# indrajeetadityaroy9/vit-inductive-bias-distillation

Hardware: AMD Instinct MI355X
Metric: distillation images/sec (BASD loss fwd+bwd+grad all-reduce), DeiT-S<-ResNet-50 @ bs256/GPU (higher is better)
Workload: dtype f32; 1 GPU; cfg2 DeiT-S<-ResNet-50 224x224; per_gpu_batch=256, global_batch=256, input_dtype=float32, layout=strided (CLS-sliced / channel-major views), backward=True, grad_allreduce_bytes=88202672, grad_allreduce=none at world size 1 (bucket packed, nothing to exchange), rank_readback=auto, readback_deferred_steps=1756, selector=basd_selector_chain mode 0, parallelism=dp1

## Files before the change

### include/basd_hip.h

```cpp
#ifndef BASD_HIP_H
#define BASD_HIP_H

#include <stdint.h>

#ifdef __cplusplus
extern "C" {
#endif

#ifndef __HIP_PLATFORM_AMD__
typedef struct ihipStream_t* hipStream_t;
#endif

#define BASD_OK 0
#define BASD_EINVAL (-1)
#define BASD_EUNSUPPORTED (-2)
#define BASD_DTYPE_F32 0
#define BASD_DTYPE_BF16 1


int basd_gemm_nt(const void* a, int a_dtype, long a_sb, long a_sn, long a_sd, int a_rows_per_batch,
                 long a_batch_stride, const float* b, long ldb, long b_batch_stride, int M, int N, int K, int batch,
                 float* c, long ldc, long c_batch_stride, float scale, const float* bias, float beta,
                 float* colsum_part, float* col_mean, hipStream_t stream);

// ... 10 lines not shown
                 int rows, int cols, int batch, int parts, float* partial, float* mean, hipStream_t stream);

int basd_gemm_tuning(int split_bf16);
int basd_gemm_tuning_get(void);

int basd_colmean_multi(const void* const* x_ptrs, int dtype, long sb, long sn, long sd, int rows_per_batch, int rows,
                       int cols, int n_mats, int parts, float* partial, float* means, int vec_ok,
                       hipStream_t stream);

int basd_syrk_splits(int krows, int cols, int n_mats);

int basd_syrk_multi(const void* const* x_ptrs, int dtype, long sb, long sn, long sd, int rows_per_batch, int krows,
                    int cols, int n_mats, const float* means, const float* scales, int splits, float* slabs,
                    float* out, long out_stride, int vec_ok, const float* fold, int fold_parts, int fold_from,
                    hipStream_t stream);


int basd_jacobi_workspace_ints(int batch, int max_sweeps);
int basd_jacobi_plain4_fits(int n);

int basd_jacobi_tuning(int lanes_per_pair);
int basd_jacobi_ordering(int odd_even);

int basd_jacobi_onesided(float* W, long batch_stride, int rows_dot, int rows_tot, int n, int batch,
                         const int* n_arr, float* colnorm, int colnorm_stride, int max_sweeps, float tol_cos,
                         int* flags, int* sweeps_out, hipStream_t stream);

long basd_jacobi_twopass_workspace_bytes(int n, int batch, int max_sweeps);
int basd_jacobi_stacked_twopass(float* W, long batch_stride, int n, int batch, float* colnorm, int colnorm_stride,
                                int max_sweeps, float tol_cos, void* workspace, int* sweeps_out, hipStream_t stream);
// ... 60 lines not shown
                              const unsigned* go_flag, unsigned go_value, int go_budget, hipStream_t stream);
int basd_flag_set(unsigned* flag, unsigned value, hipStream_t stream);

typedef struct BasdSelectorChain {
    const void* const* teacher_host_ptrs;
    long t_dtype, t_sb, t_sn, t_sd;
    const void* const* student_ptrs;
    long s_dtype, s_sb, s_sn, s_sd, s_vec_ok;
    const float* proj_t;
    const float* proj_s_t;
    long E, L, B, n_s, n_t, d_s, d_t;
    double mp_factor;
    long rank_cap;
    long kmax, kmax_cap, mode;
    float* z; float* z_sums; const void* const* z_ptrs; float* z_means; float* t_slabs; long t_splits;
    float* s_partial; float* s_means; float* s_slabs; long s_splits, s_parts;
    float* grams; float* d; float* e; float* tau; float* vh; float* vals; void* tri_work; void* tri_work_s;
    int* ranks; int* host_mirror;
    int* student_status_mirror;
    float* zv; float* vecs; float* u_rot; float* sw; float* cos; float* sigma; float* d_out;
    int* k_arr; const int* sw_index; int* jflags;
    hipStream_t main_stream, chain_stream, student_stream, tail_stream;
    void* ev_fork; void* ev_student; void* ev_ranks; void* ev_tail; void* ev_slot_free; void* ev_tgram; void* ev_tg0;
    long release_delay;
    hipStream_t fact_stream; unsigned* go_flag; long go_value; long go_budget;
    void* tm_proj; void* tm_tgram; void* tm_scol0; void* tm_scol1; void* tm_sgram; void* tm_tri0; void* tm_mid; void* tm_spec;
    hipStream_t cert_stream; int* cert_mirror; void* ev_cert;
    double* cert_scratch;
} BasdSelectorChain;
int basd_selector_chain(const BasdSelectorChain* args);
int basd_rank_certificate(const float* grams, const float* zbar, int n, int batch, double factor, double* scratch,
// ... 164 lines not shown
```

### vit-inductive-bias-distillation_amd/basd_amd/_lib.py

```python
from __future__ import annotations

import ctypes as C
import os
import threading

_HERE = os.path.dirname(os.path.abspath(__file__))
LIB_PATH = os.path.join(_HERE, "libbasd_hip.so")

vp, i32, i64, f32, f64 = C.c_void_p, C.c_int, C.c_long, C.c_float, C.c_double

SIGNATURES = {
    "basd_gemm_nt": [vp, i32, i64, i64, i64, i32, i64, vp, i64, i64, i32, i32, i32, i32, vp, i64, i64, f32, vp, f32,
                     vp, vp, vp],
    "basd_gemm_tn_splits": [i32],
    "basd_gemm_tn": [vp, vp, i32, i64, i64, i64, i64, i64, i64, i64, i64, i32, i32, i32, i32, i32, vp, vp, i32, vp,
                     vp, i64, i64, f32, vp],
    "basd_colmean_parts": [i32],
    "basd_colmean": [vp, i32, i64, i64, i64, i32, i64, i32, i32, i32, i32, vp, vp, vp],
    "basd_colmean_multi": [vp, i32, i64, i64, i64, i32, i32, i32, i32, i32, vp, vp, i32, vp],
    "basd_syrk_splits": [i32, i32, i32],
    "basd_syrk_multi": [vp, i32, i64, i64, i64, i32, i32, i32, i32, vp, vp, i32, vp, vp, i64, i32, vp, i32, i32, vp],
    "basd_jacobi_workspace_ints": [i32, i32],
    "basd_jacobi_twopass_workspace_bytes": [i32, i32, i32],
    "basd_jacobi_stacked_twopass": [vp, i64, i32, i32, vp, i32, i32, f32, vp, vp, vp],
    "basd_jacobi_tuning": [i32],
    "basd_jacobi_ordering": [i32],
    "basd_gemm_tuning": [i32],
    "basd_gemm_tuning_get": [],
    "basd_jacobi_onesided": [vp, i64, i32, i32, i32, i32, vp, vp, i32, i32, f32, vp, vp, vp],
    "basd_sort_extract": [vp, i64, i32, i32, i32, i32, vp, i32, vp, vp, i32, vp],
    "basd_tridiag_workspace_bytes": [i32, i32],
    "basd_tridiag_tuning": [i32, i32, i32, i32, i32, i32],
    "basd_tridiag": [vp, i64, i32, i32, vp, vp, vp, vp, vp, vp],
    "basd_tridiag_ranked": [vp, i64, i32, i32, vp, vp, vp, vp, vp, i32, f64, i32, vp, vp, vp, vp],
    "basd_tridiag_ranked_gated": [vp, i64, i32, i32, vp, vp, vp, vp, vp, i32, f64, i32, vp, vp, vp, C.c_uint, i32, vp],
    "basd_flag_set": [vp, C.c_uint, vp],
# ... 83 lines not shown
                             "grad_layers", "g_slabs")]
        + [("g_splits", i64)]
        + [("uw_ce", vp), ("uw_out", vp), ("jac_ws", vp), ("w_stack", vp), ("sigma_u", vp)]
    )


class SelectorChainArgs(C.Structure):
    _fields_ = (
        [("teacher_host_ptrs", vp)] + [(n, i64) for n in ("t_dtype", "t_sb", "t_sn", "t_sd")]
        + [("student_ptrs", vp)] + [(n, i64) for n in ("s_dtype", "s_sb", "s_sn", "s_sd", "s_vec_ok")]
        + [("proj_t", vp), ("proj_s_t", vp)]
        + [(n, i64) for n in ("E", "L", "B", "n_s", "n_t", "d_s", "d_t")]
        + [("mp_factor", f64)]
        + [(n, i64) for n in ("rank_cap", "kmax", "kmax_cap", "mode")]
        + [(n, vp) for n in ("z", "z_sums", "z_ptrs", "z_means", "t_slabs")] + [("t_splits", i64)]
        + [(n, vp) for n in ("s_partial", "s_means", "s_slabs")] + [("s_splits", i64), ("s_parts", i64)]
        + [(n, vp) for n in ("grams", "d", "e", "tau", "vh", "vals", "tri_work", "tri_work_s", "ranks", "host_mirror",
                             "student_status_mirror", "zv", "vecs", "u_rot", "sw", "cos", "sigma", "d_out", "k_arr",
                             "sw_index", "jflags", "main_stream", "chain_stream", "student_stream", "tail_stream",
                             "ev_fork", "ev_student", "ev_ranks", "ev_tail", "ev_slot_free", "ev_tgram", "ev_tg0",
                             "release_delay", "fact_stream", "go_flag", "go_value", "go_budget",
                             "tm_proj", "tm_tgram", "tm_scol0", "tm_scol1", "tm_sgram", "tm_tri0", "tm_mid", "tm_spec",
                             "cert_stream", "cert_mirror", "ev_cert", "cert_scratch")]
    )


EINVAL, EUNSUPPORTED = -1, -2

LONG_RESULTS = {"basd_tridiag_workspace_bytes", "basd_jacobi_twopass_workspace_bytes",
                "basd_mix_grad_tokens_scratch_floats", "basd_teacher_center_stream_scratch_floats",
                "basd_rank_certificate_scratch_bytes"}
# ... 47 lines not shown
```

### vit-inductive-bias-distillation_amd/basd_amd/chain.py

```python
from __future__ import annotations

import ctypes as C

import torch

from . import _lib, ops

import os

RELEASE_DELAY = int(os.environ.get("BASD_CHAIN_RELEASE_DELAY", "0"))
EARLY_LAUNCH = os.environ.get("BASD_CHAIN_EARLY", "0") == "1"
EARLY_BUDGET = 1500
CERTIFICATE = os.environ.get("BASD_RANK_CERT", "1") != "0"
SLOTS = max(2, int(os.environ.get("BASD_CHAIN_SLOTS", "3")))
TAIL_STREAMS = int(os.environ.get("BASD_TAIL_STREAMS", "0"))
TAIL_SPLIT_RANK = 96
SPEC_MARGIN = 8


TIMED_EVENTS = False
TM_NAMES = ("tm_proj", "tm_tgram", "tm_scol0", "tm_scol1", "tm_sgram", "tm_tri0", "tm_mid", "tm_spec")
TIMING: list | None = None


# ... 13 lines not shown
class _Slot:

    def __init__(self, plan: "SelectorChainPlan"):
        p = plan
        dev, f32, i32 = p.device, torch.float32, torch.int32
        E, L, n, K = p.E, p.L, p.d_s, p.kmax_cap
        M_t, M_s = p.B * p.n_t, p.B * p.n_s
        tiles = (M_t + 127) // 128
        nmat = 2 * L + E

        def buf(count, dtype=f32):
            return torch.empty((int(count),), device=dev, dtype=dtype)

        self.t_splits = _lib.query("basd_syrk_splits", M_t, n, L)
        self.s_splits = _lib.query("basd_syrk_splits", M_s, n, E)
        self.s_parts = _lib.query("basd_colmean_parts", M_s)
        b = self.bufs = dict(
            z=buf(L * M_t * n), z_sums=buf(L * tiles * n), z_means=buf(L * n), t_slabs=buf(L * self.t_splits * n * n),
            s_partial=buf(E * self.s_parts * n), s_means=buf(E * n), s_slabs=buf(E * self.s_splits * n * n),
            grams=buf(nmat * n * n), d=buf(nmat * n), e=buf(nmat * n), tau=buf(nmat * n), vh=buf(nmat * n * n),
            vals=buf(nmat * n), ranks=buf(L, i32),
            zv=buf((L + E) * K * n), vecs=buf((L + E) * K * n), u_rot=buf(L * K * n), sw=buf(L * K),
            cos=buf(E * L * K * K), sigma=buf(E * L * K), k_arr=buf(E * L, i32),
            jflags=buf(_lib.query("basd_jacobi_workspace_ints", E * L, ops.MAX_SWEEPS), i32),
        )
        split = p.mode not in (0, 4)
        b["tri_work"] = buf(_lib.query("basd_tridiag_workspace_bytes", n, 2 * L if split else nmat), torch.uint8)
        b["tri_work_s"] = buf(_lib.query("basd_tridiag_workspace_bytes", n, E), torch.uint8) if split else None
        b["z_ptrs"] = torch.tensor([b["z"].data_ptr() + 4 * l * M_t * n for l in range(L)], dtype=torch.int64).to(dev)
        b["sw_index"] = torch.tensor(list(range(L)) * E, dtype=i32).to(dev)
        b["go_flag"] = torch.zeros((1,), device=dev, dtype=i32)
        self.go_value = 0
        self.mirror = torch.zeros((L + 8,), dtype=i32).pin_memory()
        self.student_mirror = torch.zeros((8,), dtype=i32).pin_memory() if split else None
        self.ev_fork, self.ev_student, self.ev_ranks, self.ev_tail, self.ev_tgram, self.ev_tg0 = (_event() for _ in range(6))
        self.ev_cert = _event()
        self.cert_mirror = torch.zeros((8,), dtype=i32).pin_memory()
        self.used = False
        self.student_status_pending = False
        self.teacher_ptrs = (C.c_void_p * L)()
        self.d_out = None

        a = self.args = _lib.SelectorChainArgs()
        a.teacher_host_ptrs = C.cast(self.teacher_ptrs, C.c_void_p)
        a.E, a.L, a.B, a.n_s, a.n_t, a.d_s, a.d_t = E, L, p.B, p.n_s, p.n_t, n, p.d_t
        a.mp_factor = (1 + (n / M_t) ** 0.5) ** 2
        a.rank_cap, a.kmax_cap, a.mode = n - 1, K, p.mode
        a.t_splits, a.s_splits, a.s_parts = self.t_splits, self.s_splits, self.s_parts
        for name in ("z", "z_sums", "z_ptrs", "z_means", "t_slabs", "s_partial", "s_means", "s_slabs", "grams", "d", "e",
                     "tau", "vh", "vals", "tri_work", "tri_work_s", "ranks", "zv", "vecs", "u_rot", "sw", "cos", "sigma",
                     "k_arr", "sw_index", "jflags"):
            setattr(a, name, None if b[name] is None else b[name].data_ptr())
        a.host_mirror = self.mirror.data_ptr()
        a.student_status_mirror = None if self.student_mirror is None else self.student_mirror.data_ptr()
        a.ev_fork, a.ev_student, a.ev_ranks, a.ev_tail = self.ev_fork, self.ev_student, self.ev_ranks, self.ev_tail
        a.ev_tgram = self.ev_tgram
        a.ev_tg0 = self.ev_tg0
        a.release_delay = RELEASE_DELAY
        if p.cert_stream is not None:
            b["cert_scratch"] = torch.zeros((_lib.query("basd_rank_certificate_scratch_bytes", L),), device=dev,
                                            dtype=torch.uint8)
            a.cert_stream, a.cert_mirror, a.ev_cert = p.cert_stream.cuda_stream, self.cert_mirror.data_ptr(), self.ev_cert
            a.cert_scratch = b["cert_scratch"].data_ptr()
# ... 127 lines not shown
```

### vit-inductive-bias-distillation_amd/basd_amd/ops.py

```python
from __future__ import annotations

from dataclasses import dataclass
from functools import lru_cache

import torch

from . import _lib

import os

F32, BF16 = 0, 1
MAX_SWEEPS = 20
TWO_PASS_SVD = True
TRANSPOSED_MIX_GRAD = True
TWO_PASS_LOG_LIMIT = 16 << 30
EIG_SOLVER = os.environ.get("BASD_EIG_SOLVER", "tridiag")
if os.environ.get("BASD_GEMM_SPLIT") in ("0", "1"):
    _lib.call("basd_gemm_tuning", int(os.environ["BASD_GEMM_SPLIT"]))
if os.environ.get("BASD_JACOBI_ORDERING") in ("0", "1"):
    _lib.call("basd_jacobi_ordering", int(os.environ["BASD_JACOBI_ORDERING"]))


def _stream() -> int:
    return torch._C._cuda_getCurrentRawStream(torch._C._cuda_getDevice())
# ... 143 lines not shown
        if len(_COLMEAN_SCRATCH) >= 16:
            _COLMEAN_SCRATCH.clear()
        partial = _COLMEAN_SCRATCH[key] = torch.empty((n, parts, cols), device=dev, dtype=torch.float32)
    _lib.call("basd_colmean_multi", table.data_ptr(), dt, sb, sn, sd, rpb, rows, cols, n, parts, partial.data_ptr(),
              means.data_ptr(), vec_ok, _stream())
    return means.view(n, cols)


def centered_grams(xs: list[torch.Tensor], *, centered: list[bool] | None = None,
                   scales: list[float] | None = None, out: torch.Tensor | None = None,
                   splits: int | None = None, means: torch.Tensor | None = None,
                   fold: tuple[torch.Tensor, int] | None = None) -> tuple[torch.Tensor, torch.Tensor]:
    (dt, sb, sn, sd, rpb), rows, cols, vec_ok = _gram_layout(xs)
    n, dev = len(xs), xs[0].device
    table = _ptr_table(xs)
    if fold is not None:
        part, fold_from = fold
        assert part.is_contiguous() and part.dtype == torch.float32 and part.shape[0] == n - fold_from
        means_used = None
        centered = None
    elif means is None:
        means = column_means(xs)
    if fold is not None:
        pass
    elif centered is not None and not all(centered):
        keep = _device_consts(tuple(1.0 if c else 0.0 for c in centered), torch.float32, dev)
        means_used = means * keep.unsqueeze(1)
    else:
        means_used = means
    sc = None
# ... 594 lines not shown
```

### vit-inductive-bias-distillation_amd/csrc/chain.hip

```cpp
#include "basd_common.h"
#include "../../include/basd_hip.h"
#include <stdlib.h>

namespace basd {

__global__ void __launch_bounds__(256) chain_sw_kernel(const float* __restrict__ vals, int n, int kmax,
                                                       float* __restrict__ sw) {
    const int l = blockIdx.x;
    for (int i = threadIdx.x; i < kmax; i += 256) sw[(long)l * kmax + i] = sqrtf(fmaxf(vals[(long)l * n + i], 0.f));
}

__global__ void chain_k_arr_kernel(const int* __restrict__ ranks, int L, int items, int kmax, int* __restrict__ k_arr) {
    const int i = blockIdx.x * blockDim.x + threadIdx.x;
    if (i < items) {
        int k = ranks[i % L];
        k = k < 1 ? 1 : k;
        k_arr[i] = k > kmax ? kmax : k;
    }
}

constexpr int CERT_BLOCKS = 32;
__global__ void __launch_bounds__(256) rank_certificate_kernel(const float* __restrict__ grams, const float* __restrict__ zbar,
                                                               int n, int L, double factor, double* __restrict__ scratch,
                                                               int* __restrict__ host_flag) {
// ... 244 lines not shown
    }
    BASD_TRY(basd_syrk_multi(a->z_ptrs, BASD_DTYPE_F32, 0, n, 1, 1 << 30, (int)M_t, n, L, a->z_means, nullptr,
                             (int)a->t_splits, a->t_slabs, a->grams + (long)L * nn, nn, 1, nullptr, 0, 0, cs));
    BASD_TRY(basd_gram_finish(a->grams + (long)L * nn, a->z_means, n, L, M_t, a->grams, nullptr, cs));
    BASD_MARK(a->tm_tgram, cs);
    if (mode == 3) BASD_CHECK_ARG(a->ev_tg0 != nullptr);
    if (a->ev_tg0) BASD_HIP(hipEventRecord((hipEvent_t)a->ev_tg0, cs));
    if (a->cert_mirror) {
        BASD_CHECK_ARG(a->cert_stream && a->ev_cert && a->ev_tg0 && a->cert_scratch);
        if (a->cert_stream != cs) BASD_HIP(hipStreamWaitEvent(a->cert_stream, (hipEvent_t)a->ev_tg0, 0));
        BASD_TRY(basd_rank_certificate(a->grams, a->z_means, n, L, a->mp_factor, a->cert_scratch, a->cert_mirror, a->cert_stream));
        BASD_HIP(hipEventRecord((hipEvent_t)a->ev_cert, a->cert_stream));
    }

    auto student_grams = [&](hipStream_t st) -> int {
        BASD_MARK(a->tm_scol0, st);
        BASD_TRY(basd_colmean_multi(a->student_ptrs, (int)a->s_dtype, a->s_sb, a->s_sn, a->s_sd, n_s, (int)M_s, n, E,
                                    (int)a->s_parts, a->s_partial, a->s_means, (int)a->s_vec_ok, st));
        BASD_MARK(a->tm_scol1, st);
        BASD_TRY(basd_syrk_multi(a->student_ptrs, (int)a->s_dtype, a->s_sb, a->s_sn, a->s_sd, n_s, (int)M_s, n, E,
                                 a->s_means, nullptr, (int)a->s_splits, a->s_slabs, a->grams + 2L * L * nn, nn,
                                 (int)a->s_vec_ok, nullptr, 0, 0, st));
        BASD_MARK(a->tm_sgram, st);
        return BASD_OK;
    };

    if (mode == 0 || mode == 4) {
        BASD_TRY(student_grams(ss));
        if (ss != cs) {
            BASD_HIP(hipEventRecord((hipEvent_t)a->ev_student, ss));
            BASD_HIP(hipStreamWaitEvent(cs, (hipEvent_t)a->ev_student, 0));
        }
        BASD_MARK(a->tm_tri0, cs);
        BASD_TRY(basd_tridiag_ranked(a->grams, nn, n, 2 * L + E, a->d, a->e, a->tau, a->vh, a->tri_work, L, a->mp_factor,
                                     (int)a->rank_cap, a->ranks, a->host_mirror, a->tm_mid, cs));
        BASD_HIP(hipEventRecord((hipEvent_t)a->ev_ranks, cs));
    } else {
// ... 29 lines not shown
```

### vit-inductive-bias-distillation_amd/csrc/gemm.hip

```cpp
#include "basd_common.h"

namespace basd {

typedef float f32x16 __attribute__((ext_vector_type(16)));

constexpr int BM = 128, BN = 128;

typedef __bf16 bf16x8 __attribute__((ext_vector_type(8)));

__device__ __forceinline__ unsigned cvt_pk_bf16(float a, float b) {
    unsigned r;
    asm("v_cvt_pk_bf16_f32 %0, %1, %2" : "=v"(r) : "v"(a), "v"(b));
    return r;
}

__device__ __forceinline__ void split3(float a, float b, unsigned& hi, unsigned& mid, unsigned& lo) {
    hi = cvt_pk_bf16(a, b);
    const float ra = a - __uint_as_float(hi << 16), rb = b - __uint_as_float(hi & 0xffff0000u);
    mid = cvt_pk_bf16(ra, rb);
    const float sa = ra - __uint_as_float(mid << 16), sb = rb - __uint_as_float(mid & 0xffff0000u);
    lo = cvt_pk_bf16(sa, sb);
}


// ... 519 lines not shown
                    acc[mi][ni] = __builtin_amdgcn_mfma_f32_32x32x2f32(a[mi].w, b[ni].w, acc[mi][ni], 0, 0, 0);
                }
        }
    }
    store_tile(C, ldc, M, N, m0, n0, acc, wm, wn, lane, scale);
}


__device__ __forceinline__ void tri_tile(int p, int& mi, int& ni) {
    mi = 0;
    while ((mi + 1) * (mi + 2) / 2 <= p) ++mi;
    ni = p - mi * (mi + 1) / 2;
}

template <typename T, bool VEC>
__global__ void __launch_bounds__(256) syrk_tn_kernel(const void* const* __restrict__ ptrs, GemmOperand X, int cols,
                                                      int Krows, int splits, int n_mats, int pairs,
                                                      const float* __restrict__ means, float* __restrict__ slabs,
                                                      const float* __restrict__ fold, int fold_parts, int fold_from) {
    __shared__ __attribute__((aligned(16))) float lds[2 * TN_BK * 128];
    int pair, unit;
    {
        const int units = splits * n_mats, id = blockIdx.x;
        if ((units & 7) == 0) {
            const int xcd = id & 7, slot = id >> 3;
            pair = slot % pairs;
            unit = xcd + 8 * (slot / pairs);
        } else {
            pair = id % pairs;
            unit = id / pairs;
        }
    }
    int tmi, tni;
    tri_tile(pair, tmi, tni);
// ... 26 lines not shown
    const int col0 = is_b ? n0 : m0;
    float* tile = is_b ? tB : tA;
    float reg[2][4][4], m4[4];
    TnCursor cu;
    tn_cursor_init(cu, X, k_begin, t);
    if (fold && z >= fold_from) {
        const float* fp = fold + (long)(z - fold_from) * fold_parts * cols;
        const int c = col0 + (t & 31) * 4;
#pragma unroll
        for (int e = 0; e < 4; ++e) {
            float s = 0.f;
            if (c + e < cols)
                for (int p = 0; p < fold_parts; ++p) s += fp[(long)p * cols + c + e];
            m4[e] = s * (1.f / Krows);
        }
    } else {
        tn_mean4(mean, cols, col0, t, m4);
    }
    if (loader && k_begin < k_end) tn_load<T, VEC>(X, cu, k_end, cols, k_begin, col0, t, m4, reg);
    const int i = lane & 31, h = lane >> 5;
    for (int k0 = k_begin; k0 < k_end; k0 += TN_BK) {
        __syncthreads();
        if (loader) tn_store_lds(tile, t, reg, m4);
        __syncthreads();
        if (loader && k0 + TN_BK < k_end) {
            tn_cursor_advance(cu, X);
            tn_load<T, VEC>(X, cu, k_end, cols, k0 + TN_BK, col0, t, m4, reg);
        }
#pragma unroll
        for (int g = 0; g < TN_BK / 8; ++g) {
            float4 a[2], b[2];
#pragma unroll
            for (int mi = 0; mi < 2; ++mi) a[mi] = *(const float4*)(tA + (((2 * g + h) * 128 + wm * 64 + mi * 32 + i) << 2));
#pragma unroll
            for (int ni = 0; ni < 2; ++ni) b[ni] = *(const float4*)(tB + (((2 * g + h) * 128 + wn * 64 + ni * 32 + i) << 2));
#pragma unroll
            for (int mi = 0; mi < 2; ++mi)
#pragma unroll
                for (int ni = 0; ni < 2; ++ni) {
                    acc[mi][ni] = __builtin_amdgcn_mfma_f32_32x32x2f32(a[mi].x, b[ni].x, acc[mi][ni], 0, 0, 0);
                    acc[mi][ni] = __builtin_amdgcn_mfma_f32_32x32x2f32(a[mi].y, b[ni].y, acc[mi][ni], 0, 0, 0);
                    acc[mi][ni] = __builtin_amdgcn_mfma_f32_32x32x2f32(a[mi].z, b[ni].z, acc[mi][ni], 0, 0, 0);
                    acc[mi][ni] = __builtin_amdgcn_mfma_f32_32x32x2f32(a[mi].w, b[ni].w, acc[mi][ni], 0, 0, 0);
                }
        }
    }
    store_tile(C, cols, cols, cols, m0, n0, acc, wm, wn, lane, 1.f);
}

constexpr int SPLIT_PLANE = (TN_BK / 8) * 128 * 8;

__device__ __forceinline__ void tn_store_lds_split(unsigned short* __restrict__ tile, int t, const float (&reg)[2][4][4],
                                                   const float (&m4)[4]) {
    const int l = t & 31;
#pragma unroll
    for (int j = 0; j < 2; ++j) {
        const int kg = (t >> 5) + 4 * j, o = kg >> 1, half = kg & 1;
#pragma unroll
        for (int e = 0; e < 4; ++e) {
            unsigned h0, m0, l0, h1, m1, l1;
            split3(reg[j][0][e] - m4[e], reg[j][1][e] - m4[e], h0, m0, l0);
            split3(reg[j][2][e] - m4[e], reg[j][3][e] - m4[e], h1, m1, l1);
            unsigned short* p = tile + ((o * 128 + 32 * e + l) << 3) + 4 * half;
            *(uint2*)(p) = make_uint2(h0, h1);
            *(uint2*)(p + SPLIT_PLANE) = make_uint2(m0, m1);
            *(uint2*)(p + 2 * SPLIT_PLANE) = make_uint2(l0, l1);
        }
    }
}

template <typename T, bool VEC>
__global__ void __launch_bounds__(256) syrk_tn_split_kernel(const void* const* __restrict__ ptrs, GemmOperand X, int cols,
                                                            int Krows, int splits, int n_mats, int pairs,
                                                            const float* __restrict__ means, float* __restrict__ slabs,
                                                            const float* __restrict__ fold, int fold_parts, int fold_from) {
    __shared__ __attribute__((aligned(16))) unsigned short lds[2 * 3 * SPLIT_PLANE];
    int pair, unit;
    {
        const int units = splits * n_mats, id = blockIdx.x;
        if ((units & 7) == 0) {
            const int xcd = id & 7, slot = id >> 3;
            pair = slot % pairs;
            unit = xcd + 8 * (slot / pairs);
        } else {
            pair = id % pairs;
            unit = id / pairs;
        }
    }
    int tmi, tni;
    tri_tile(pair, tmi, tni);
// ... 26 lines not shown
    const int col0 = is_b ? n0 : m0;
    unsigned short* tile = is_b ? tB : tA;
    float reg[2][4][4], m4[4];
    TnCursor cu;
    tn_cursor_init(cu, X, k_begin, t);
    if (fold && z >= fold_from) {
        const float* fp = fold + (long)(z - fold_from) * fold_parts * cols;
        const int c = col0 + (t & 31) * 4;
#pragma unroll
        for (int e = 0; e < 4; ++e) {
            float s = 0.f;
            if (c + e < cols)
                for (int p = 0; p < fold_parts; ++p) s += fp[(long)p * cols + c + e];
            m4[e] = s * (1.f / Krows);
        }
    } else {
        tn_mean4(mean, cols, col0, t, m4);
    }
    if (loader && k_begin < k_end) tn_load<T, VEC>(X, cu, k_end, cols, k_begin, col0, t, m4, reg);
    const int i = lane & 31, h = lane >> 5;
    for (int k0 = k_begin; k0 < k_end; k0 += TN_BK) {
        __syncthreads();
        if (loader) tn_store_lds_split(tile, t, reg, m4);
        __syncthreads();
        if (loader && k0 + TN_BK < k_end) {
            tn_cursor_advance(cu, X);
            tn_load<T, VEC>(X, cu, k_end, cols, k0 + TN_BK, col0, t, m4, reg);
        }
#pragma unroll
        for (int s16 = 0; s16 < TN_BK / 16; ++s16) {
            bf16x8 a[2][3], b[2][3];
            const int o = 2 * s16 + h;
#pragma unroll
            for (int mi = 0; mi < 2; ++mi)
#pragma unroll
                for (int p = 0; p < 3; ++p)
                    a[mi][p] = *(const bf16x8*)(tA + p * SPLIT_PLANE + ((o * 128 + (wm * 2 + mi) * 32 + i) << 3));
#pragma unroll
// ... 16 lines not shown
                }
        }
    }
#pragma unroll
    for (int mi = 0; mi < 2; ++mi)
#pragma unroll
        for (int ni = 0; ni < 2; ++ni) {
            const int col = n0 + 4 * i + (wn * 2 + ni);
            if (col >= cols) continue;
#pragma unroll
            for (int r = 0; r < 16; ++r) {
                const int row = m0 + 4 * ((r & 3) + 8 * (r >> 2) + 4 * h) + (wm * 2 + mi);
                if (row < cols) C[(long)row * cols + col] = acc[mi][ni][r];
            }
        }
}

template <typename T, bool VEC>
__global__ void __launch_bounds__(256) gemm_tn_split_kernel(GemmOperand A, GemmOperand B, int M, int N, int Krows,
                                                            int splits, const float* __restrict__ mean_a,
                                                            const float* __restrict__ mean_b, float* __restrict__ C,
                                                            long ldc, long c_z_stride, float scale) {
    __shared__ __attribute__((aligned(16))) unsigned short lds[2 * 3 * SPLIT_PLANE];
    unsigned short* tA = lds;
    unsigned short* tB = lds + 3 * SPLIT_PLANE;
    const int tid = threadIdx.x, lane = tid & 63, wave = tid >> 6, wm = wave >> 1, wn = wave & 1;
    const int m0 = blockIdx.y * BM, n0 = blockIdx.x * BN;
    const int bz = blockIdx.z / splits, sp = blockIdx.z - bz * splits;
    A.ptr = (const T*)A.ptr + (long)bz * A.batch_stride;
    B.ptr = (const T*)B.ptr + (long)bz * B.batch_stride;
// ... 65 lines not shown
    for (int mi = 0; mi < 2; ++mi)
#pragma unroll
        for (int ni = 0; ni < 2; ++ni) {
            const int col = n0 + 4 * i + (wn * 2 + ni);
            if (col >= N) continue;
#pragma unroll
            for (int r = 0; r < 16; ++r) {
                const int row = m0 + 4 * ((r & 3) + 8 * (r >> 2) + 4 * h) + (wm * 2 + mi);
                if (row < M) C[(long)row * ldc + col] = acc[mi][ni][r] * scale;
            }
        }
}

__global__ void __launch_bounds__(256) syrk_reduce_kernel(const float* __restrict__ slabs, int cols, int splits,
                                                          const float* __restrict__ scales, float* __restrict__ out,
                                                          long out_stride) {
    int tmi, tni;
    tri_tile(blockIdx.x >> 6, tmi, tni);
    const int e = (blockIdx.x & 63) * 256 + threadIdx.x;
    const int r = tmi * BM + (e >> 7), c = tni * BN + (e & 127);
    if (r >= cols || c >= cols) return;
    const int z = blockIdx.y;
    const long mat = (long)cols * cols;
    const bool up = tmi == tni && r < c;
    const float* in = slabs + (long)z * splits * mat + (up ? (long)c * cols + r : (long)r * cols + c);
    float s = 0.f;
    for (int k = 0; k < splits; ++k) s += in[k * mat];
    s *= scales ? scales[z] : 1.f;
    float* o = out + (long)z * out_stride;
    o[(long)r * cols + c] = s;
    if (tmi != tni) o[(long)c * cols + r] = s;
}

__global__ void reduce_slabs_kernel(const float* __restrict__ slabs, long slab_stride, int splits, long count,
                                    float scale, float* __restrict__ out, long batch_in_stride,
                                    long batch_out_stride) {
    const float* in = slabs + (long)blockIdx.y * batch_in_stride;
    float* o = out + (long)blockIdx.y * batch_out_stride;
    for (long i = (long)blockIdx.x * blockDim.x + threadIdx.x; i < count; i += (long)gridDim.x * blockDim.x) {
        float s = 0.f;
        for (int k = 0; k < splits; ++k) s += in[(long)k * slab_stride + i];
        o[i] = s * scale;
// ... 232 lines not shown
    if (cap < 1) cap = 1;
    const double slots = 768.0;
    auto fill = [&](int s) {
        const double x = (double)(w * s) / slots;
        const double rounds = x <= 1.0 ? 1.0 : (double)(long)(x + 0.999999);
        return x / rounds;
    };
    double best_eff = 0.0;
    for (int s = 1; s <= cap; ++s) best_eff = fill(s) > best_eff ? fill(s) : best_eff;
    int best = cap;
    for (int s = 1; s <= cap; ++s)
        if (fill(s) >= 0.97 * best_eff) { best = s; break; }
    return best;
}

int basd_syrk_multi(const void* const* x_ptrs, int dtype, long sb, long sn, long sd, int rows_per_batch, int krows,
                    int cols, int n_mats, const float* means, const float* scales, int splits, float* slabs,
                    float* out, long out_stride, int vec_ok, const float* fold, int fold_parts, int fold_from,
                    hipStream_t stream) {
    BASD_CHECK_ARG(x_ptrs && slabs && out && krows > 0 && cols > 0 && n_mats > 0 && splits >= 1 && rows_per_batch > 0);
    BASD_CHECK_ARG(out_stride >= (long)cols * cols);
    BASD_CHECK_ARG(!fold || (fold_parts > 0 && fold_from >= 0 && fold_from <= n_mats));
    GemmOperand X{nullptr, sb, sn, sd, rows_per_batch, 0};
    const int tiles = (cols + BM - 1) / BM, pairs = tiles * (tiles + 1) / 2;
    const dim3 grid(pairs * splits * n_mats);
    if (g_gemm_split && dtype == BASD_DTYPE_F32) {
        const bool vec = vec_ok && sd == 1 && sb % 4 == 0 && sn % 4 == 0;
        if (vec) syrk_tn_split_kernel<float, true><<<grid, 256, 0, stream>>>(x_ptrs, X, cols, krows, splits, n_mats, pairs, means, slabs, fold, fold_parts, fold_from);
        else syrk_tn_split_kernel<float, false><<<grid, 256, 0, stream>>>(x_ptrs, X, cols, krows, splits, n_mats, pairs, means, slabs, fold, fold_parts, fold_from);
    } else if (g_gemm_split && dtype == BASD_DTYPE_BF16) {
        if (sd == 1) syrk_tn_split_kernel<__hip_bfloat16, true><<<grid, 256, 0, stream>>>(x_ptrs, X, cols, krows, splits, n_mats, pairs, means, slabs, fold, fold_parts, fold_from);
        else syrk_tn_split_kernel<__hip_bfloat16, false><<<grid, 256, 0, stream>>>(x_ptrs, X, cols, krows, splits, n_mats, pairs, means, slabs, fold, fold_parts, fold_from);
    } else if (dtype == BASD_DTYPE_F32) {
        const bool vec = vec_ok && sd == 1 && sb % 4 == 0 && sn % 4 == 0;
        if (vec) syrk_tn_kernel<float, true><<<grid, 256, 0, stream>>>(x_ptrs, X, cols, krows, splits, n_mats, pairs, means, slabs, fold, fold_parts, fold_from);
        else syrk_tn_kernel<float, false><<<grid, 256, 0, stream>>>(x_ptrs, X, cols, krows, splits, n_mats, pairs, means, slabs, fold, fold_parts, fold_from);
    } else if (dtype == BASD_DTYPE_BF16) {
        if (sd == 1) syrk_tn_kernel<__hip_bfloat16, true><<<grid, 256, 0, stream>>>(x_ptrs, X, cols, krows, splits, n_mats, pairs, means, slabs, fold, fold_parts, fold_from);
        else syrk_tn_kernel<__hip_bfloat16, false><<<grid, 256, 0, stream>>>(x_ptrs, X, cols, krows, splits, n_mats, pairs, means, slabs, fold, fold_parts, fold_from);
    } else {
        return BASD_EINVAL;
    }
    syrk_reduce_kernel<<<dim3(pairs * 64, n_mats), 256, 0, stream>>>(slabs, cols, splits, scales, out, out_stride);
    BASD_RETURN_LAST();
}

int basd_colmean_multi(const void* const* x_ptrs, int dtype, long sb, long sn, long sd, int rows_per_batch, int rows,
                       int cols, int n_mats, int parts, float* partial, float* means, int vec_ok,
                       hipStream_t stream) {
    BASD_CHECK_ARG(x_ptrs && partial && means && rows > 0 && cols > 0 && n_mats > 0 && parts >= 1);
    GemmOperand X{nullptr, sb, sn, sd, rows_per_batch, 0};
    const int esz = dtype == BASD_DTYPE_F32 ? 4 : 2;
    const bool vec = vec_ok && sd == 1 && cols % 4 == 0 && (sb * esz) % 16 == 0 && (sn * esz) % 16 == 0;
    if (dtype == BASD_DTYPE_F32) launch_colsum<float>(X, x_ptrs, nullptr, rows, cols, parts, n_mats, vec, partial, stream);
    else if (dtype == BASD_DTYPE_BF16) launch_colsum<__hip_bfloat16>(X, x_ptrs, nullptr, rows, cols, parts, n_mats, vec, partial, stream);
    else return BASD_EINVAL;
    colsum_final_kernel<<<dim3((cols + 63) / 64, n_mats), 256, 0, stream>>>(partial, cols, parts, 1.f / rows, means);
    BASD_RETURN_LAST();
}
// ... 3 lines not shown
```

Measured before the change: 167,100 images/s.

## Fuse student column-mean pass into shifted SYRK with rank-one centring correction

```diff
diff --git a/include/basd_hip.h b/include/basd_hip.h
--- a/include/basd_hip.h
+++ b/include/basd_hip.h
@@ -48,6 +48,11 @@
                     int cols, int n_mats, const float* means, const float* scales, int splits, float* slabs,
                     float* out, long out_stride, int vec_ok, const float* fold, int fold_parts, int fold_from,
                     hipStream_t stream);
+
+int basd_syrk_centred_multi(const void* const* x_ptrs, int dtype, long sb, long sn, long sd, int rows_per_batch,
+                            int krows, int cols, int n_mats, const float* scales, int splits, float* slabs,
+                            double* colpart, float* out, long out_stride, float* means_out, int vec_ok,
+                            hipStream_t stream);
 
 
 int basd_jacobi_workspace_ints(int batch, int max_sweeps);
@@ -138,7 +143,7 @@
     long rank_cap;
     long kmax, kmax_cap, mode;
     float* z; float* z_sums; const void* const* z_ptrs; float* z_means; float* t_slabs; long t_splits;
-    float* s_partial; float* s_means; float* s_slabs; long s_splits, s_parts;
+    double* s_partial; float* s_means; float* s_slabs; long s_splits;
     float* grams; float* d; float* e; float* tau; float* vh; float* vals; void* tri_work; void* tri_work_s;
     int* ranks; int* host_mirror;
     int* student_status_mirror;
diff --git a/vit-inductive-bias-distillation_amd/basd_amd/_lib.py b/vit-inductive-bias-distillation_amd/basd_amd/_lib.py
--- a/vit-inductive-bias-distillation_amd/basd_amd/_lib.py
+++ b/vit-inductive-bias-distillation_amd/basd_amd/_lib.py
@@ -20,6 +20,7 @@
     "basd_colmean_multi": [vp, i32, i64, i64, i64, i32, i32, i32, i32, i32, vp, vp, i32, vp],
     "basd_syrk_splits": [i32, i32, i32],
     "basd_syrk_multi": [vp, i32, i64, i64, i64, i32, i32, i32, i32, vp, vp, i32, vp, vp, i64, i32, vp, i32, i32, vp],
+    "basd_syrk_centred_multi": [vp, i32, i64, i64, i64, i32, i32, i32, i32, vp, i32, vp, vp, vp, i64, vp, i32, vp],
     "basd_jacobi_workspace_ints": [i32, i32],
     "basd_jacobi_twopass_workspace_bytes": [i32, i32, i32],
     "basd_jacobi_stacked_twopass": [vp, i64, i32, i32, vp, i32, i32, f32, vp, vp, vp],
@@ -133,7 +134,7 @@
         + [("mp_factor", f64)]
         + [(n, i64) for n in ("rank_cap", "kmax", "kmax_cap", "mode")]
         + [(n, vp) for n in ("z", "z_sums", "z_ptrs", "z_means", "t_slabs")] + [("t_splits", i64)]
-        + [(n, vp) for n in ("s_partial", "s_means", "s_slabs")] + [("s_splits", i64), ("s_parts", i64)]
+        + [(n, vp) for n in ("s_partial", "s_means", "s_slabs")] + [("s_splits", i64)]
         + [(n, vp) for n in ("grams", "d", "e", "tau", "vh", "vals", "tri_work", "tri_work_s", "ranks", "host_mirror",
                              "student_status_mirror", "zv", "vecs", "u_rot", "sw", "cos", "sigma", "d_out", "k_arr",
                              "sw_index", "jflags", "main_stream", "chain_stream", "student_stream", "tail_stream",
diff --git a/vit-inductive-bias-distillation_amd/basd_amd/chain.py b/vit-inductive-bias-distillation_amd/basd_amd/chain.py
--- a/vit-inductive-bias-distillation_amd/basd_amd/chain.py
+++ b/vit-inductive-bias-distillation_amd/basd_amd/chain.py
@@ -51,10 +51,9 @@
 
         self.t_splits = _lib.query("basd_syrk_splits", M_t, n, L)
         self.s_splits = _lib.query("basd_syrk_splits", M_s, n, E)
-        self.s_parts = _lib.query("basd_colmean_parts", M_s)
         b = self.bufs = dict(
             z=buf(L * M_t * n), z_sums=buf(L * tiles * n), z_means=buf(L * n), t_slabs=buf(L * self.t_splits * n * n),
-            s_partial=buf(E * self.s_parts * n), s_means=buf(E * n), s_slabs=buf(E * self.s_splits * n * n),
+            s_partial=buf(E * (self.s_splits + 1) * n, torch.float64), s_means=buf(E * n), s_slabs=buf(E * self.s_splits * n * n),
             grams=buf(nmat * n * n), d=buf(nmat * n), e=buf(nmat * n), tau=buf(nmat * n), vh=buf(nmat * n * n),
             vals=buf(nmat * n), ranks=buf(L, i32),
             zv=buf((L + E) * K * n), vecs=buf((L + E) * K * n), u_rot=buf(L * K * n), sw=buf(L * K),
@@ -83,7 +82,7 @@
         a.E, a.L, a.B, a.n_s, a.n_t, a.d_s, a.d_t = E, L, p.B, p.n_s, p.n_t, n, p.d_t
         a.mp_factor = (1 + (n / M_t) ** 0.5) ** 2
         a.rank_cap, a.kmax_cap, a.mode = n - 1, K, p.mode
-        a.t_splits, a.s_splits, a.s_parts = self.t_splits, self.s_splits, self.s_parts
+        a.t_splits, a.s_splits = self.t_splits, self.s_splits
         for name in ("z", "z_sums", "z_ptrs", "z_means", "t_slabs", "s_partial", "s_means", "s_slabs", "grams", "d", "e",
                      "tau", "vh", "vals", "tri_work", "tri_work_s", "ranks", "zv", "vecs", "u_rot", "sw", "cos", "sigma",
                      "k_arr", "sw_index", "jflags"):
diff --git a/vit-inductive-bias-distillation_amd/basd_amd/ops.py b/vit-inductive-bias-distillation_amd/basd_amd/ops.py
--- a/vit-inductive-bias-distillation_amd/basd_amd/ops.py
+++ b/vit-inductive-bias-distillation_amd/basd_amd/ops.py
@@ -181,6 +181,20 @@
     (dt, sb, sn, sd, rpb), rows, cols, vec_ok = _gram_layout(xs)
     n, dev = len(xs), xs[0].device
     table = _ptr_table(xs)
+    if fold is None and means is None and (centered is None or all(centered)):
+        sc = _device_consts(tuple(float(s) for s in scales), torch.float32, dev) if scales is not None else None
+        if splits is None:
+            splits = _lib.query("basd_syrk_splits", rows, cols, n)
+        slabs = torch.empty((n * splits, cols, cols), device=dev, dtype=torch.float32)
+        colpart = torch.empty((n, splits + 1, cols), device=dev, dtype=torch.float64)
+        means = torch.empty((n, cols), device=dev, dtype=torch.float32)
+        if out is None:
+            out = torch.empty((n, cols, cols), device=dev, dtype=torch.float32)
+        assert out.dtype == torch.float32 and out.shape == (n, cols, cols) and out[0].is_contiguous()
+        _lib.call("basd_syrk_centred_multi", table.data_ptr(), dt, sb, sn, sd, rpb, rows, cols, n, _ptr(sc), splits,
+                  slabs.data_ptr(), colpart.data_ptr(), out.data_ptr(), out.stride(0), means.data_ptr(), vec_ok,
+                  _stream())
+        return out, means
     if fold is not None:
         part, fold_from = fold
         assert part.is_contiguous() and part.dtype == torch.float32 and part.shape[0] == n - fold_from
diff --git a/vit-inductive-bias-distillation_amd/csrc/chain.hip b/vit-inductive-bias-distillation_amd/csrc/chain.hip
--- a/vit-inductive-bias-distillation_amd/csrc/chain.hip
+++ b/vit-inductive-bias-distillation_amd/csrc/chain.hip
@@ -282,13 +282,10 @@
     }
 
     auto student_grams = [&](hipStream_t st) -> int {
-        BASD_MARK(a->tm_scol0, st);
-        BASD_TRY(basd_colmean_multi(a->student_ptrs, (int)a->s_dtype, a->s_sb, a->s_sn, a->s_sd, n_s, (int)M_s, n, E,
-                                    (int)a->s_parts, a->s_partial, a->s_means, (int)a->s_vec_ok, st));
         BASD_MARK(a->tm_scol1, st);
-        BASD_TRY(basd_syrk_multi(a->student_ptrs, (int)a->s_dtype, a->s_sb, a->s_sn, a->s_sd, n_s, (int)M_s, n, E,
-                                 a->s_means, nullptr, (int)a->s_splits, a->s_slabs, a->grams + 2L * L * nn, nn,
-                                 (int)a->s_vec_ok, nullptr, 0, 0, st));
+        BASD_TRY(basd_syrk_centred_multi(a->student_ptrs, (int)a->s_dtype, a->s_sb, a->s_sn, a->s_sd, n_s, (int)M_s, n, E,
+                                         nullptr, (int)a->s_splits, a->s_slabs, a->s_partial, a->grams + 2L * L * nn, nn,
+                                         a->s_means, (int)a->s_vec_ok, st));
         BASD_MARK(a->tm_sgram, st);
         return BASD_OK;
     };
diff --git a/vit-inductive-bias-distillation_amd/csrc/gemm.hip b/vit-inductive-bias-distillation_amd/csrc/gemm.hip
--- a/vit-inductive-bias-distillation_amd/csrc/gemm.hip
+++ b/vit-inductive-bias-distillation_amd/csrc/gemm.hip
@@ -557,10 +557,63 @@
 }
 
 template <typename T, bool VEC>
+__device__ __forceinline__ void syrk_shift4(const GemmOperand& X, int Krows, int cols, int col0, int t, bool is_b,
+                                            bool loader, float* __restrict__ red, float (&m4)[4]) {
+    float* r = red + (is_b ? 512 : 0);
+    const int c = (t & 31) * 4;
+    if (loader) {
+        const float zero[4] = {0.f, 0.f, 0.f, 0.f};
+        float reg[2][4][4];
+        TnCursor c0;
+        tn_cursor_init(c0, X, 0, t);
+        tn_load<T, VEC>(X, c0, Krows, cols, 0, col0, t, zero, reg);
+#pragma unroll
+        for (int e = 0; e < 4; ++e)
+            r[(t >> 5) * 128 + c + e] = ((reg[0][0][e] + reg[0][1][e]) + (reg[0][2][e] + reg[0][3][e])) +
+                                        ((reg[1][0][e] + reg[1][1][e]) + (reg[1][2][e] + reg[1][3][e]));
+    }
+    __syncthreads();
+    const float inv = 1.f / (float)(Krows < TN_BK ? Krows : TN_BK);
+#pragma unroll
+    for (int e = 0; e < 4; ++e)
+        m4[e] = loader ? ((r[c + e] + r[128 + c + e]) + (r[256 + c + e] + r[384 + c + e])) * inv : 0.f;
+}
+
+__device__ __forceinline__ void syrk_colsum_acc(double (&cs)[4], const float (&reg)[2][4][4], const float (&m4)[4]) {
+#pragma unroll
+    for (int e = 0; e < 4; ++e)
+        cs[e] += (double)(((reg[0][0][e] - m4[e]) + (reg[0][1][e] - m4[e])) + ((reg[0][2][e] - m4[e]) + (reg[0][3][e] - m4[e])) +
+                          (((reg[1][0][e] - m4[e]) + (reg[1][1][e] - m4[e])) + ((reg[1][2][e] - m4[e]) + (reg[1][3][e] - m4[e]))));
+}
+
+__device__ __forceinline__ void syrk_colsum_out(const double (&cs)[4], const float (&m4)[4], double* __restrict__ red,
+                                                int tid, int cols, int col0, int z, int sp, int splits,
+                                                double* __restrict__ colpart) {
+    __syncthreads();
+    const int c = (tid & 31) * 4;
+    if (tid < 128) {
+#pragma unroll
+        for (int e = 0; e < 4; ++e) red[(tid >> 5) * 128 + c + e] = cs[e];
+    }
+    __syncthreads();
+    if (tid < 32) {
+        double* o = colpart + (long)z * (splits + 1) * cols;
+#pragma unroll
+        for (int e = 0; e < 4; ++e) {
+            const int cc = col0 + c + e;
+            if (cc >= cols) continue;
+            o[(long)sp * cols + cc] = (red[c + e] + red[128 + c + e]) + (red[256 + c + e] + red[384 + c + e]);
+            if (sp == 0) o[(long)splits * cols + cc] = (double)m4[e];
+        }
+    }
+}
+
+template <typename T, bool VEC>
 __global__ void __launch_bounds__(256) syrk_tn_kernel(const void* const* __restrict__ ptrs, GemmOperand X, int cols,
                                                       int Krows, int splits, int n_mats, int pairs,
                                                       const float* __restrict__ means, float* __restrict__ slabs,
-                                                      const float* __restrict__ fold, int fold_parts, int fold_from) {
+                                                      const float* __restrict__ fold, int fold_parts, int fold_from,
+                                                      double* __restrict__ colpart) {
     __shared__ __attribute__((aligned(16))) float lds[2 * TN_BK * 128];
     int pair, unit;
     {
@@ -617,14 +670,19 @@
                 for (int p = 0; p < fold_parts; ++p) s += fp[(long)p * cols + c + e];
             m4[e] = s * (1.f / Krows);
         }
+    } else if (colpart) {
+        syrk_shift4<T, VEC>(X, Krows, cols, col0, t, is_b, loader, lds, m4);
     } else {
         tn_mean4(mean, cols, col0, t, m4);
     }
+    const bool sums = colpart && diag;
+    double cs[4] = {0.0, 0.0, 0.0, 0.0};
     if (loader && k_begin < k_end) tn_load<T, VEC>(X, cu, k_end, cols, k_begin, col0, t, m4, reg);
     const int i = lane & 31, h = lane >> 5;
     for (int k0 = k_begin; k0 < k_end; k0 += TN_BK) {
         __syncthreads();
         if (loader) tn_store_lds(tile, t, reg, m4);
+        if (sums && loader) syrk_colsum_acc(cs, reg, m4);
         __syncthreads();
         if (loader && k0 + TN_BK < k_end) {
             tn_cursor_advance(cu, X);
@@ -649,6 +707,7 @@
         }
     }
     store_tile(C, cols, cols, cols, m0, n0, acc, wm, wn, lane, 1.f);
+    if (sums) syrk_colsum_out(cs, m4, (double*)lds, tid, cols, col0, z, sp, splits, colpart);
 }
 
 constexpr int SPLIT_PLANE = (TN_BK / 8) * 128 * 8;
@@ -676,7 +735,8 @@
 __global__ void __launch_bounds__(256) syrk_tn_split_kernel(const void* const* __restrict__ ptrs, GemmOperand X, int cols,
                                                             int Krows, int splits, int n_mats, int pairs,
                                                             const float* __restrict__ means, float* __restrict__ slabs,
-                                                            const float* __restrict__ fold, int fold_parts, int fold_from) {
+                                                            const float* __restrict__ fold, int fold_parts, int fold_from,
+                                                            double* __restrict__ colpart) {
     __shared__ __attribute__((aligned(16))) unsigned short lds[2 * 3 * SPLIT_PLANE];
     int pair, unit;
     {
@@ -733,14 +793,19 @@
                 for (int p = 0; p < fold_parts; ++p) s += fp[(long)p * cols + c + e];
             m4[e] = s * (1.f / Krows);
         }
+    } else if (colpart) {
+        syrk_shift4<T, VEC>(X, Krows, cols, col0, t, is_b, loader, (float*)lds, m4);
     } else {
         tn_mean4(mean, cols, col0, t, m4);
     }
+    const bool sums = colpart && diag;
+    double cs[4] = {0.0, 0.0, 0.0, 0.0};
     if (loader && k_begin < k_end) tn_load<T, VEC>(X, cu, k_end, cols, k_begin, col0, t, m4, reg);
     const int i = lane & 31, h = lane >> 5;
     for (int k0 = k_begin; k0 < k_end; k0 += TN_BK) {
         __syncthreads();
         if (loader) tn_store_lds_split(tile, t, reg, m4);
+        if (sums && loader) syrk_colsum_acc(cs, reg, m4);
         __syncthreads();
         if (loader && k0 + TN_BK < k_end) {
             tn_cursor_advance(cu, X);
@@ -787,6 +852,7 @@
                 if (row < cols) C[(long)row * cols + col] = acc[mi][ni][r];
             }
         }
+    if (sums) syrk_colsum_out(cs, m4, (double*)lds, tid, cols, col0, z, sp, splits, colpart);
 }
 
 template <typename T, bool VEC>
@@ -882,18 +948,42 @@
 
 __global__ void __launch_bounds__(256) syrk_reduce_kernel(const float* __restrict__ slabs, int cols, int splits,
                                                           const float* __restrict__ scales, float* __restrict__ out,
-                                                          long out_stride) {
+                                                          long out_stride, const double* __restrict__ colpart, int krows,
+                                                          float* __restrict__ means_out) {
+    __shared__ double dcol[128], drow[2];
     int tmi, tni;
     tri_tile(blockIdx.x >> 6, tmi, tni);
     const int e = (blockIdx.x & 63) * 256 + threadIdx.x;
     const int r = tmi * BM + (e >> 7), c = tni * BN + (e & 127);
+    const int z = blockIdx.y;
+    if (colpart) {
+        const double* cp = colpart + (long)z * (splits + 1) * cols;
+        const int tid = threadIdx.x;
+        const int j = tid < 128 ? tni * BN + tid : tmi * BM + ((blockIdx.x & 63) * 256 >> 7) + (tid - 128);
+        if (tid < 130) {
+            double s = 0.0;
+            if (j < cols)
+                for (int k = 0; k < splits; ++k) s += cp[(long)k * cols + j];
+            s /= (double)krows;
+            if (tid < 128) dcol[tid] = s;
+            else drow[tid - 128] = s;
+            if (means_out && tmi == tni && (blockIdx.x & 63) == 0 && tid < 128 && j < cols)
+                means_out[(long)z * cols + j] = (float)(cp[(long)splits * cols + j] + s);
+        }
+        __syncthreads();
+    }
     if (r >= cols || c >= cols) return;
-    const int z = blockIdx.y;
     const long mat = (long)cols * cols;
     const bool up = tmi == tni && r < c;
-    const float* in = slabs + (long)z * splits * mat + (up ? (long)c * cols + r : (long)r * cols + c);
+    const int rr = up ? c : r, cc = up ? r : c;
+    const float* in = slabs + (long)z * splits * mat + (long)rr * cols + cc;
     float s = 0.f;
     for (int k = 0; k < splits; ++k) s += in[k * mat];
+    if (colpart) {
+        const double d_r = tmi == tni ? dcol[rr - tni * BN] : drow[threadIdx.x >> 7];
+        const double d_c = dcol[cc - tni * BN];
+        s = (float)((double)s - (d_r * d_c) * (double)krows);
+    }
     s *= scales ? scales[z] : 1.f;
     float* o = out + (long)z * out_stride;
     o[(long)r * cols + c] = s;
@@ -1156,35 +1246,56 @@
     return best;
 }
 
+static int syrk_launch(const void* const* x_ptrs, int dtype, long sb, long sn, long sd, int rows_per_batch, int krows,
+                       int cols, int n_mats, const float* means, const float* scales, int splits, float* slabs,
+                       float* out, long out_stride, int vec_ok, const float* fold, int fold_parts, int fold_from,
+                       double* colpart, float* means_out, hipStream_t stream) {
+    BASD_CHECK_ARG(x_ptrs && slabs && out && krows > 0 && cols > 0 && n_mats > 0 && splits >= 1 && rows_per_batch > 0);
+    BASD_CHECK_ARG(out_stride >= (long)cols * cols);
+    BASD_CHECK_ARG(!fold || (fold_parts > 0 && fold_from >= 0 && fold_from <= n_mats));
+    BASD_CHECK_ARG(!colpart || (!means && !fold));
+    GemmOperand X{nullptr, sb, sn, sd, rows_per_batch, 0};
+    const int tiles = (cols + BM - 1) / BM, pairs = tiles * (tiles + 1) / 2;
+    const dim3 grid(pairs * splits * n_mats);
+#define SYRK_ARGS x_ptrs, X, cols, krows, splits, n_mats, pairs, means, slabs, fold, fold_parts, fold_from, colpart
+    if (g_gemm_split && dtype == BASD_DTYPE_F32) {
+        const bool vec = vec_ok && sd == 1 && sb % 4 == 0 && sn % 4 == 0;
+        if (vec) syrk_tn_split_kernel<float, true><<<grid, 256, 0, stream>>>(SYRK_ARGS);
+        else syrk_tn_split_kernel<float, false><<<grid, 256, 0, stream>>>(SYRK_ARGS);
+    } else if (g_gemm_split && dtype == BASD_DTYPE_BF16) {
+        if (sd == 1) syrk_tn_split_kernel<__hip_bfloat16, true><<<grid, 256, 0, stream>>>(SYRK_ARGS);
+        else syrk_tn_split_kernel<__hip_bfloat16, false><<<grid, 256, 0, stream>>>(SYRK_ARGS);
+    } else if (dtype == BASD_DTYPE_F32) {
+        const bool vec = vec_ok && sd == 1 && sb % 4 == 0 && sn % 4 == 0;
+        if (vec) syrk_tn_kernel<float, true><<<grid, 256, 0, stream>>>(SYRK_ARGS);
+        else syrk_tn_kernel<float, false><<<grid, 256, 0, stream>>>(SYRK_ARGS);
+    } else if (dtype == BASD_DTYPE_BF16) {
+        if (sd == 1) syrk_tn_kernel<__hip_bfloat16, true><<<grid, 256, 0, stream>>>(SYRK_ARGS);
+        else syrk_tn_kernel<__hip_bfloat16, false><<<grid, 256, 0, stream>>>(SYRK_ARGS);
+    } else {
+        return BASD_EINVAL;
+    }
+#undef SYRK_ARGS
+    syrk_reduce_kernel<<<dim3(pairs * 64, n_mats), 256, 0, stream>>>(slabs, cols, splits, scales, out, out_stride, colpart,
+                                                                     krows, means_out);
+    BASD_RETURN_LAST();
+}
+
 int basd_syrk_multi(const void* const* x_ptrs, int dtype, long sb, long sn, long sd, int rows_per_batch, int krows,
                     int cols, int n_mats, const float* means, const float* scales, int splits, float* slabs,
                     float* out, long out_stride, int vec_ok, const float* fold, int fold_parts, int fold_from,
                     hipStream_t stream) {
-    BASD_CHECK_ARG(x_ptrs && slabs && out && krows > 0 && cols > 0 && n_mats > 0 && splits >= 1 && rows_per_batch > 0);
-    BASD_CHECK_ARG(out_stride >= (long)cols * cols);
-    BASD_CHECK_ARG(!fold || (fold_parts > 0 && fold_from >= 0 && fold_from <= n_mats));
-    GemmOperand X{nullptr, sb, sn, sd, rows_per_batch, 0};
-    const int tiles = (cols + BM - 1) / BM, pairs = tiles * (tiles + 1) / 2;
-    const dim3 grid(pairs * splits * n_mats);
-    if (g_gemm_split && dtype == BASD_DTYPE_F32) {
-        const bool vec = vec_ok && sd == 1 && sb % 4 == 0 && sn % 4 == 0;
-        if (vec) syrk_tn_split_kernel<float, true><<<grid, 256, 0, stream>>>(x_ptrs, X, cols, krows, splits, n_mats, pairs, means, slabs, fold, fold_parts, fold_from);
-        else syrk_tn_split_kernel<float, false><<<grid, 256, 0, stream>>>(x_ptrs, X, cols, krows, splits, n_mats, pairs, means, slabs, fold, fold_parts, fold_from);
-    } else if (g_gemm_split && dtype == BASD_DTYPE_BF16) {
-        if (sd == 1) syrk_tn_split_kernel<__hip_bfloat16, true><<<grid, 256, 0, stream>>>(x_ptrs, X, cols, krows, splits, n_mats, pairs, means, slabs, fold, fold_parts, fold_from);
-        else syrk_tn_split_kernel<__hip_bfloat16, false><<<grid, 256, 0, stream>>>(x_ptrs, X, cols, krows, splits, n_mats, pairs, means, slabs, fold, fold_parts, fold_from);
-    } else if (dtype == BASD_DTYPE_F32) {
-        const bool vec = vec_ok && sd == 1 && sb % 4 == 0 && sn % 4 == 0;
-        if (vec) syrk_tn_kernel<float, true><<<grid, 256, 0, stream>>>(x_ptrs, X, cols, krows, splits, n_mats, pairs, means, slabs, fold, fold_parts, fold_from);
-        else syrk_tn_kernel<float, false><<<grid, 256, 0, stream>>>(x_ptrs, X, cols, krows, splits, n_mats, pairs, means, slabs, fold, fold_parts, fold_from);
-    } else if (dtype == BASD_DTYPE_BF16) {
-        if (sd == 1) syrk_tn_kernel<__hip_bfloat16, true><<<grid, 256, 0, stream>>>(x_ptrs, X, cols, krows, splits, n_mats, pairs, means, slabs, fold, fold_parts, fold_from);
-        else syrk_tn_kernel<__hip_bfloat16, false><<<grid, 256, 0, stream>>>(x_ptrs, X, cols, krows, splits, n_mats, pairs, means, slabs, fold, fold_parts, fold_from);
-    } else {
-        return BASD_EINVAL;
-    }
-    syrk_reduce_kernel<<<dim3(pairs * 64, n_mats), 256, 0, stream>>>(slabs, cols, splits, scales, out, out_stride);
-    BASD_RETURN_LAST();
+    return syrk_launch(x_ptrs, dtype, sb, sn, sd, rows_per_batch, krows, cols, n_mats, means, scales, splits, slabs, out,
+                       out_stride, vec_ok, fold, fold_parts, fold_from, nullptr, nullptr, stream);
+}
+
+int basd_syrk_centred_multi(const void* const* x_ptrs, int dtype, long sb, long sn, long sd, int rows_per_batch,
+                            int krows, int cols, int n_mats, const float* scales, int splits, float* slabs,
+                            double* colpart, float* out, long out_stride, float* means_out, int vec_ok,
+                            hipStream_t stream) {
+    BASD_CHECK_ARG(colpart != nullptr);
+    return syrk_launch(x_ptrs, dtype, sb, sn, sd, rows_per_batch, krows, cols, n_mats, nullptr, scales, splits, slabs,
+                       out, out_stride, vec_ok, nullptr, 0, 0, colpart, means_out, stream);
 }
 
 int basd_colmean_multi(const void* const* x_ptrs, int dtype, long sb, long sn, long sd, int rows_per_batch, int rows,
```

New measurement: 164,100 images/s (median of 2 runs). No clear change (-1.8%).
